# HenryHZY/VL-PET

Hardware: AMD Instinct MI355X
Metric: multitask samples/sec (BART-base, r=96) (higher is better)
Workload: dtype bf16

## Files before the change

vl-pet_amd/csrc/attn.hip:

```cpp
#include <cstdlib>
#include "common.h"
#include "kernels.h"

#define AT_LD 72
#define AT_ROW (AT_LD * 2)
#define AT_NW 4
#define LOG2E 1.4426950408889634f

typedef short v4s16_t __attribute__((ext_vector_type(4)));
typedef short v8s16_t __attribute__((ext_vector_type(8)));

__device__ __forceinline__ float fast_exp2(float x) { return __builtin_amdgcn_exp2f(x); }

__device__ __forceinline__ uint32_t hash32(uint32_t x) {
    x ^= x >> 16; x *= 0x7feb352dU; x ^= x >> 15; x *= 0x846ca68bU; x ^= x >> 16;
    return x;
}
__device__ __forceinline__ uint32_t row_key(uint64_t seed, int64_t row) {
    const uint32_t k = hash32((uint32_t)seed ^ hash32((uint32_t)(seed >> 32) + (uint32_t)((uint64_t)row >> 32)));
    return hash32(k + (uint32_t)row);
}
__device__ __forceinline__ uint32_t hash_elem(uint32_t x) {
    x ^= x >> 16; x *= 0x7feb352dU; x ^= x >> 15;
    return __builtin_amdgcn_alignbit(x, x, 16) * 0x846ca68bU;
}
__device__ __forceinline__ bool keep_elem(uint32_t rk, int j, uint32_t thr) { return hash_elem(rk + (uint32_t)j * 0x9E3779B9U) >= thr; }

__device__ __forceinline__ bf16x8 tr_acc_order(const uint8_t* img, int kb, int cb, int lane) {
    const int g = lane >> 4, sl = lane & 15;
    const uint8_t* p = img + (size_t)(kb + 4 * (g >> 1) + (sl >> 2)) * AT_ROW + (cb + 16 * (g & 1) + 4 * (sl & 3)) * 2;
    typedef __attribute__((address_space(3))) v4s16_t lds_v4;
    const v4s16_t lo = __builtin_amdgcn_ds_read_tr16_b64_v4i16((lds_v4*)(p));
    const v4s16_t hi = __builtin_amdgcn_ds_read_tr16_b64_v4i16((lds_v4*)(p + 8 * AT_ROW));
    const v8s16_t r = {lo[0], lo[1], lo[2], lo[3], hi[0], hi[1], hi[2], hi[3]};
    return __builtin_bit_cast(bf16x8, r);
}
__device__ __forceinline__ bf16x8 nat_frag(const uint8_t* img, int row, int ks, int hh) {
    return *reinterpret_cast<const bf16x8*>(img + (size_t)row * AT_ROW + (16 * ks + 8 * hh) * 2);
}
__device__ __forceinline__ bf16x8 acc_frag(const f32x16& t, int u) {
    bf16x8 f;
#pragma unroll
    for (int j = 0; j < 8; ++j) f[j] = (__bf16)t[8 * u + j];
    return f;
}
__device__ __forceinline__ void stage_image(uint8_t* img, const __bf16* src, int64_t rs, int n_rows, int rows_pad, int tid, int nthreads) {
    const u32x4 z = {0u, 0u, 0u, 0u};
    for (int idx = tid; idx < rows_pad * 8; idx += nthreads) {
        const int row = idx >> 3, pc = idx & 7;
        u32x4 v = z;
        if (row < n_rows) v = __builtin_nontemporal_load(reinterpret_cast<const u32x4*>(src + (int64_t)row * rs + pc * 8));
        *reinterpret_cast<u32x4*>(img + (size_t)row * AT_ROW + pc * 16) = v;
    }
}
template <int NIMG, int MAXP>
__device__ __forceinline__ void stage_images(uint8_t* const* img, const __bf16* const* src, const int* n_rows, const int* rows_pad,
                                             const int64_t* rs, int tid, int nthreads) {
    u32x4 v[NIMG][MAXP];
#pragma unroll
    for (int g = 0; g < NIMG; ++g)
#pragma unroll
        for (int c = 0; c < MAXP; ++c) {
            const int idx = tid + c * nthreads, row = idx >> 3, pc = idx & 7;
            const int rr = row < n_rows[g] ? row : n_rows[g] - 1;
            v[g][c] = __builtin_nontemporal_load(reinterpret_cast<const u32x4*>(src[g] + (int64_t)rr * rs[g] + pc * 8));
        }
    const u32x4 z = {0u, 0u, 0u, 0u};
#pragma unroll
    for (int g = 0; g < NIMG; ++g)
#pragma unroll
        for (int c = 0; c < MAXP; ++c) {
            const int idx = tid + c * nthreads, row = idx >> 3, pc = idx & 7;
            if (row < rows_pad[g]) *reinterpret_cast<u32x4*>(img[g] + (size_t)row * AT_ROW + pc * 16) = row < n_rows[g] ? v[g][c] : z;
        }
}
#define AT_SROW 144
#define AT_STG (16 * AT_SROW)
__device__ __forceinline__ void store_rows_T(uint8_t* stg, const f32x16& t0, const f32x16& t1, __bf16* dst, int64_t rs,
                                             int row0, int n_rows, int lane) {
    const int m = lane & 31, hh = lane >> 5;
    typedef __bf16 bf16x4_t __attribute__((ext_vector_type(4)));
#pragma unroll
    for (int half = 0; half < 2; ++half) {
        if ((m >> 4) == half) {
#pragma unroll
            for (int dt = 0; dt < 2; ++dt) {
                const f32x16& t = dt ? t1 : t0;
#pragma unroll
                for (int q = 0; q < 4; ++q) {
                    bf16x4_t w;
#pragma unroll
                    for (int e = 0; e < 4; ++e) w[e] = (__bf16)t[4 * q + e];
                    *reinterpret_cast<bf16x4_t*>(stg + (size_t)(m & 15) * AT_SROW + (32 * dt + 8 * q + 4 * hh) * 2) = w;
                }
            }
        }
        asm volatile("" ::: "memory");
        u32x4 v[2];
#pragma unroll
        for (int c = 0; c < 2; ++c) {
            const int idx = lane + 64 * c, row = idx >> 3, pc = idx & 7;
            v[c] = *reinterpret_cast<const u32x4*>(stg + (size_t)row * AT_SROW + pc * 16);
        }
        asm volatile("" ::: "memory");
#pragma unroll
        for (int c = 0; c < 2; ++c) {
            const int idx = lane + 64 * c, row = 16 * half + (idx >> 3), pc = idx & 7;
            if (row0 + row < n_rows) *reinterpret_cast<u32x4*>(dst + (int64_t)(row0 + row) * rs + pc * 8) = v[c];
        }
    }
}

__device__ __forceinline__ f32x16 bias_tile(const float* brow, float inv_scale) {
    f32x16 t;
#pragma unroll
    for (int q4 = 0; q4 < 4; ++q4) {
        const f32x4 bv = *reinterpret_cast<const f32x4*>(brow + 8 * q4);
#pragma unroll
        for (int e = 0; e < 4; ++e) t[4 * q4 + e] = bv[e] * inv_scale;
    }
    return t;
}

#define AT_FW 2

struct AttnLds {
    __host__ __device__ static constexpr size_t fwd_wave_bytes(int Lkp) { return (size_t)Lkp * AT_ROW + (size_t)AT_STG + (size_t)Lkp * 4; }
    static size_t fwd_bytes(int Lkp) { return (size_t)AT_FW * fwd_wave_bytes(Lkp); }
    static size_t bwd_bytes(int Lqp, int Lkp) {
        return bwd_bytes_nw(Lqp, Lkp, AT_NW);
    }
    static size_t bwd_bytes_nw(int Lqp, int Lkp, int nw) {
        return (size_t)2 * (Lqp + Lkp) * AT_ROW + (size_t)nw * AT_STG + (size_t)Lqp * 12 + (size_t)Lkp * 4;
    }
};

__device__ __forceinline__ float key_bias(const AttnArgs& a, const uint8_t* km, int key) {
    return (key < a.Lk && (km == nullptr || km[key] != 0)) ? 0.f : -INFINITY;
}

template <int T, bool BIAS>
__global__ __launch_bounds__(AT_FW * 64, (T <= 2 ? 3 : 2)) void attn_fwd_kernel(AttnArgs a) {
    extern __shared__ __attribute__((aligned(16))) uint8_t smem[];
    const int tid = threadIdx.x, lane = tid & 63, wave = __builtin_amdgcn_readfirstlane(tid >> 6);
    const int bh = blockIdx.x * AT_FW + wave;
    if (bh >= a.B * a.H) return;
    const uint64_t seed = a.thr ? vlpet_eff_seed(a.seed, a.seed_ctr) : 0;
    const int b = bh / a.H, h = bh % a.H;
    const int m = lane & 31, hh = lane >> 5;
    constexpr int Lkp = 32 * T;
    const int64_t rs = (int64_t)a.H * 64, rq = a.ld_q, rk = a.ld_kv, rv = a.ld_v;
    const __bf16* qb_ = a.q + (int64_t)b * a.Lq * rq + h * 64;
    const __bf16* kb_ = a.k + (int64_t)b * a.Lk * rk + h * 64;
    const __bf16* vb_ = a.v + (int64_t)b * a.Lk * rv + h * 64;
    __bf16* ob_ = a.o + (int64_t)b * a.Lq * rs + h * 64;
    const uint8_t* km = a.key_mask ? a.key_mask + (int64_t)b * a.Lk : nullptr;
    uint8_t* Vs = smem + (size_t)wave * AttnLds::fwd_wave_bytes(Lkp);
    uint8_t* stg = Vs + (size_t)Lkp * AT_ROW;
    float* kval = reinterpret_cast<float*>(stg + AT_STG);
#pragma unroll
    for (int c = 0; c < (Lkp + 63) / 64; ++c)
        if (lane + 64 * c < Lkp) kval[lane + 64 * c] = key_bias(a, km, lane + 64 * c);
    const int coff = a.causal ? a.Lk - a.Lq : (1 << 20);

    bf16x8 kf[T][4];
#pragma unroll
    for (int t = 0; t < T; ++t) {
        const int j = 32 * t + m, jk = j < a.Lk ? j : a.Lk - 1;
#pragma unroll
        for (int ks = 0; ks < 4; ++ks) kf[t][ks] = *reinterpret_cast<const bf16x8*>(kb_ + (int64_t)jk * rk + 16 * ks + 8 * hh);
    }
    stage_image(Vs, vb_, rv, a.Lk, Lkp, lane, 64);

    const float sc2 = a.scale * LOG2E;
    const int NQB = (a.Lq + 31) >> 5;
    for (int qb = 0; qb < NQB; ++qb) {
        const int i = 32 * qb + m;
        const int iq = i < a.Lq ? i : a.Lq - 1;
        bf16x8 qf[4];
#pragma unroll
        for (int ks = 0; ks < 4; ++ks) qf[ks] = *reinterpret_cast<const bf16x8*>(qb_ + (int64_t)iq * rq + 16 * ks + 8 * hh);
        f32x16 st[T];
#pragma unroll
        for (int t = 0; t < T; ++t) {
            if constexpr (BIAS) st[t] = bias_tile(a.bias + ((int64_t)h * (32 * NQB) + i) * Lkp + 32 * t + 4 * hh, 1.0f / a.scale);
            else st[t] = zero16();
#pragma unroll
            for (int ks = 0; ks < 4; ++ks) st[t] = mfma32(kf[t][ks], qf[ks], st[t]);
        }
        float mx = -INFINITY;
        const int ic = i + coff - 4 * hh;
#pragma unroll
        for (int t = 0; t < T; ++t) {
#pragma unroll
            for (int q4 = 0; q4 < 4; ++q4) {
                const f32x4 kv = *reinterpret_cast<const f32x4*>(kval + 32 * t + 8 * q4 + 4 * hh);
#pragma unroll
                for (int e = 0; e < 4; ++e) {
                    const int r = 4 * q4 + e;
                    float s = fmaf(st[t][r], sc2, kv[e]);
                    s = 32 * t + e + 8 * q4 > ic ? -INFINITY : s;
                    st[t][r] = s;
                    mx = fmaxf(mx, s);
                }
            }
        }
        mx = fmaxf(mx, __shfl_xor(mx, 32));
        if (mx == -INFINITY) mx = 0.f;
        float sum = 0.f;
#pragma unroll
        for (int t = 0; t < T; ++t) {
#pragma unroll
            for (int r = 0; r < 16; ++r) { const float p = fast_exp2(st[t][r] - mx); st[t][r] = p; sum += p; }
        }
        sum += __shfl_xor(sum, 32);
        const float inv = sum > 0.f ? 1.0f / sum : 0.f;
        if (hh == 0 && i < a.Lq) a.lse[((int64_t)b * a.H + h) * a.Lq + i] = sum > 0.f ? mx + log2f(sum) : INFINITY;
        const uint32_t rk = row_key(seed, ((int64_t)b * a.H + h) * a.Lq + iq);
        const float inv_keep = a.thr ? a.inv_keep : 1.0f;
        f32x16 ot0 = zero16(), ot1 = zero16();
#pragma unroll
        for (int t = 0; t < T; ++t) {
            if (a.keep_out != nullptr && a.thr != 0) {
#pragma unroll
                for (int r = 0; r < 16; ++r) {
                    const int key = 32 * t + (r & 3) + 8 * (r >> 2) + 4 * hh;
                    if (i < a.Lq && key < a.Lk)
                        a.keep_out[(((int64_t)b * a.H + h) * a.Lq + i) * a.Lk + key] = keep_elem(rk, key, a.thr) ? 1 : 0;
                }
            }
            const uint32_t kg0 = rk + (uint32_t)(32 * t + 4 * hh) * 0x9E3779B9U;
#pragma unroll
            for (int r = 0; r < 16; ++r) {
                const int ir = (r & 3) + 8 * (r >> 2);
                const bool kp = hash_elem(kg0 + (uint32_t)ir * 0x9E3779B9U) >= a.thr;
                st[t][r] = kp ? st[t][r] * inv * inv_keep : 0.f;
            }
#pragma unroll
            for (int u = 0; u < 2; ++u) {
                const bf16x8 pf = acc_frag(st[t], u);
                ot0 = mfma32(tr_acc_order(Vs, 32 * t + 16 * u, 0, lane), pf, ot0);
                ot1 = mfma32(tr_acc_order(Vs, 32 * t + 16 * u, 32, lane), pf, ot1);
            }
        }
        store_rows_T(stg, ot0, ot1, ob_, rs, 32 * qb, a.Lq, lane);
    }
}

enum { IMG_Q = 0, IMG_D = 1, IMG_K = 2, IMG_V = 3 };
struct BwdCtx {
    const float* rowt;
    const float* kval;
    int Lqp;
    float sc2, scale, inv_keep;
    uint32_t thr;
    int coff;
};
__device__ __forceinline__ BwdCtx bwd_ctx(const AttnArgs& a, const float* rowt, const float* kval, int Lqp) {
    BwdCtx c;
    c.rowt = rowt; c.kval = kval; c.Lqp = Lqp;
    c.sc2 = a.scale * LOG2E; c.scale = a.scale; c.inv_keep = a.thr ? a.inv_keep : 1.0f; c.thr = a.thr;
    c.coff = a.causal ? a.Lk - a.Lq : (1 << 20);
    return c;
}

template <class R, bool BIAS>
__device__ __forceinline__ void bwd_k_unit(const AttnArgs& a, const BwdCtx& c, const R& rd0, int t, int NQB, int Lqp, int Lkp, int h, int lane,
                                           f32x16& dv0, f32x16& dv1, f32x16& dk0, f32x16& dk1) {
    const int m = lane & 31, hh = lane >> 5;
    const int key = 32 * t + m;
    const float kb = c.kval[key];
    const uint32_t kg = (uint32_t)key * 0x9E3779B9U;
    const int kc = key - c.coff - 4 * hh;
    for (int qb = 0; qb < NQB; ++qb) {
        const R rd = rd0.fresh();
        f32x16 s, dp = zero16();
        if constexpr (BIAS) s = bias_tile(a.bias_t + ((int64_t)h * Lkp + key) * Lqp + 32 * qb + 4 * hh, 1.0f / a.scale);
        else s = zero16();
#pragma unroll
        for (int ks = 0; ks < 4; ++ks) {
            s = mfma32(rd.nat(IMG_Q, qb, ks), rd.nat(IMG_K, t, ks), s);
            dp = mfma32(rd.nat(IMG_D, qb, ks), rd.nat(IMG_V, t, ks), dp);
        }
        const int kcq = kc - 32 * qb;
        const float* rtp = c.rowt + 32 * qb + 4 * hh;
#pragma unroll
        for (int q4 = 0; q4 < 4; ++q4) {
            __builtin_amdgcn_sched_barrier(0);
            const f32x4 ls = *reinterpret_cast<const f32x4*>(rtp + 8 * q4);
            const f32x4 dl = *reinterpret_cast<const f32x4*>(rtp + c.Lqp + 8 * q4);
            const f32x4 rk = *reinterpret_cast<const f32x4*>(rtp + 2 * c.Lqp + 8 * q4);
#pragma unroll
            for (int e = 0; e < 4; ++e) {
                const int r = 4 * q4 + e, ir = e + 8 * q4;
                float x = fmaf(s[r], c.sc2, kb - ls[e]);
                x = kcq > ir ? -INFINITY : x;
                const float p = fast_exp2(x);
                const bool kp = hash_elem(__float_as_uint(rk[e]) + kg) >= c.thr;
                const float g = kp ? dp[r] * c.inv_keep : 0.f;
                s[r] = kp ? p * c.inv_keep : 0.f;
                dp[r] = p * (g - dl[e]) * c.scale;
            }
        }
#pragma unroll
        for (int u = 0; u < 2; ++u) {
            const bf16x8 pf = acc_frag(s, u), sf = acc_frag(dp, u);
            dv0 = mfma32(rd.tr(IMG_D, 2 * qb + u, 0), pf, dv0);
            dv1 = mfma32(rd.tr(IMG_D, 2 * qb + u, 1), pf, dv1);
            dk0 = mfma32(rd.tr(IMG_Q, 2 * qb + u, 0), sf, dk0);
            dk1 = mfma32(rd.tr(IMG_Q, 2 * qb + u, 1), sf, dk1);
        }
    }
}
template <class R, bool BIAS>
__device__ __forceinline__ void bwd_q_unit(const AttnArgs& a, const BwdCtx& c, const R& rd0, int qb, int T, int Lqp, int Lkp, int h, int lane,
                                           f32x16& dq0, f32x16& dq1) {
    const int m = lane & 31, hh = lane >> 5;
    const int i = 32 * qb + m;
    bf16x8 qf[4], df[4];
#pragma unroll
    for (int ks = 0; ks < 4; ++ks) { qf[ks] = rd0.nat(IMG_Q, qb, ks); df[ks] = rd0.nat(IMG_D, qb, ks); }
    const float l2 = c.rowt[i], dl = c.rowt[c.Lqp + i];
    const uint32_t rkey = __float_as_uint(c.rowt[2 * c.Lqp + i]);
    const int ic = i + c.coff - 4 * hh;
    for (int t = 0; t < T; ++t) {
        const R rd = rd0.fresh();
        f32x16 s, dp = zero16();
        if constexpr (BIAS) s = bias_tile(a.bias + ((int64_t)h * Lqp + i) * Lkp + 32 * t + 4 * hh, 1.0f / a.scale);
        else s = zero16();
#pragma unroll
        for (int ks = 0; ks < 4; ++ks) {
            s = mfma32(rd.nat(IMG_K, t, ks), qf[ks], s);
            dp = mfma32(rd.nat(IMG_V, t, ks), df[ks], dp);
        }
        const float* kvp = c.kval + 32 * t + 4 * hh;
        const uint32_t kg0 = rkey + (uint32_t)(32 * t + 4 * hh) * 0x9E3779B9U;
        const int ict = ic - 32 * t;
#pragma unroll
        for (int q4 = 0; q4 < 4; ++q4) {
            __builtin_amdgcn_sched_barrier(0);
            const f32x4 kv = *reinterpret_cast<const f32x4*>(kvp + 8 * q4);
#pragma unroll
            for (int e = 0; e < 4; ++e) {
                const int r = 4 * q4 + e, ir = e + 8 * q4;
                float x = fmaf(s[r], c.sc2, kv[e] - l2);
                x = ir > ict ? -INFINITY : x;
                const float p = fast_exp2(x);
                const bool kp = hash_elem(kg0 + (uint32_t)ir * 0x9E3779B9U) >= c.thr;
                const float g = kp ? dp[r] * c.inv_keep : 0.f;
                dp[r] = p * (g - dl) * c.scale;
            }
        }
#pragma unroll
        for (int u = 0; u < 2; ++u) {
            const bf16x8 sf = acc_frag(dp, u);
            dq0 = mfma32(rd.tr(IMG_K, 2 * t + u, 0), sf, dq0);
            dq1 = mfma32(rd.tr(IMG_K, 2 * t + u, 1), sf, dq1);
        }
    }
}
struct PadRd {
    const uint8_t* img[4];
    int m, hh, lane;
    __device__ __forceinline__ PadRd fresh() const { PadRd r = *this; asm volatile("" : "+v"(r.m), "+v"(r.lane)); return r; }
    __device__ __forceinline__ bf16x8 nat(int im, int tile, int ks) const { return nat_frag(img[im], 32 * tile + m, ks, hh); }
    __device__ __forceinline__ bf16x8 tr(int im, int g16, int dt) const { return tr_acc_order(img[im], 16 * g16, 32 * dt, lane); }
};
template <int OCC, int NW = AT_NW, bool BIAS = false>
__global__ __launch_bounds__(NW * 64, OCC) void attn_bwd_kernel(AttnArgs a) {
    extern __shared__ __attribute__((aligned(16))) uint8_t smem[];
    const int bh = blockIdx.x, b = bh / a.H, h = bh % a.H;
    const int tid = threadIdx.x, lane = tid & 63, wave = __builtin_amdgcn_readfirstlane(tid >> 6);
    const uint64_t seed = a.thr ? vlpet_eff_seed(a.seed, a.seed_ctr) : 0;
    const int m = lane & 31, hh = lane >> 5;
    const int Lkp = (a.Lk + 31) & ~31, T = Lkp >> 5;
    const int Lqp = (a.Lq + 31) & ~31, NQB = Lqp >> 5;
    const int64_t rs = (int64_t)a.H * 64, rq = a.ld_q, rk = a.ld_kv, rv = a.ld_v;
    const int64_t ooff = (int64_t)b * a.Lq * rs + h * 64;
    const int64_t qoff = (int64_t)b * a.Lq * rq + h * 64, koff = (int64_t)b * a.Lk * rk + h * 64;
    const int64_t voff = (int64_t)b * a.Lk * rv + h * 64;
    const uint8_t* km = a.key_mask ? a.key_mask + (int64_t)b * a.Lk : nullptr;
    uint8_t* Qs = smem;
    uint8_t* Ds = Qs + (size_t)Lqp * AT_ROW;
    uint8_t* Ks = Ds + (size_t)Lqp * AT_ROW;
    uint8_t* Vs = Ks + (size_t)Lkp * AT_ROW;
    uint8_t* stg = Vs + (size_t)Lkp * AT_ROW + (size_t)wave * AT_STG;
    float* rowt = reinterpret_cast<float*>(Vs + (size_t)Lkp * AT_ROW + (size_t)NW * AT_STG);
    float* kval = rowt + 3 * Lqp;

    {
        bf16x8 xo[2][2], xd[2][2];
#pragma unroll
        for (int c = 0; c < 2; ++c) {
            const int idx = tid + c * NW * 64, row = idx >> 2, part = idx & 3;
            const int rr = row < a.Lq ? row : a.Lq - 1;
#pragma unroll
            for (int e = 0; e < 2; ++e) {
                xo[c][e] = __builtin_nontemporal_load(reinterpret_cast<const bf16x8*>(a.o + ooff + (int64_t)rr * rs + 16 * part + 8 * e));
                xd[c][e] = __builtin_nontemporal_load(reinterpret_cast<const bf16x8*>(a.dout + ooff + (int64_t)rr * rs + 16 * part + 8 * e));
            }
        }
        if (tid < Lkp) kval[tid] = key_bias(a, km, tid);
        uint8_t* const imgs[4] = {Qs, Ds, Ks, Vs};
        const __bf16* const srcs[4] = {a.q + qoff, a.dout + ooff, a.k + koff, a.v + voff};
        const int nr[4] = {a.Lq, a.Lq, a.Lk, a.Lk}, rp[4] = {Lqp, Lqp, Lkp, Lkp};
        const int64_t rss[4] = {rq, rs, rk, rv};
        stage_images<4, (NW == 6 ? 3 : 4)>(imgs, srcs, nr, rp, rss, tid, NW * 64);
#pragma unroll
        for (int c = 0; c < 2; ++c) {
            const int idx = tid + c * NW * 64, row = idx >> 2, part = idx & 3;
            float acc = 0.f;
#pragma unroll
            for (int e = 0; e < 2; ++e)
#pragma unroll
                for (int j = 0; j < 8; ++j) acc += (float)xo[c][e][j] * (float)xd[c][e][j];
            acc += __shfl_xor(acc, 1);
            acc += __shfl_xor(acc, 2);
            if (part == 0 && row < Lqp) {
                const bool live = row < a.Lq;
                rowt[row] = live ? a.lse[((int64_t)b * a.H + h) * a.Lq + row] : INFINITY;
                rowt[Lqp + row] = live ? acc : 0.f;
                rowt[2 * Lqp + row] = __uint_as_float(row_key(seed, ((int64_t)b * a.H + h) * a.Lq + (live ? row : a.Lq - 1)));
            }
        }
    }
    __syncthreads();

    const BwdCtx c = bwd_ctx(a, rowt, kval, Lqp);
    PadRd rd;
    rd.img[IMG_Q] = Qs; rd.img[IMG_D] = Ds; rd.img[IMG_K] = Ks; rd.img[IMG_V] = Vs;
    rd.m = m; rd.hh = hh; rd.lane = lane;
    for (int un = (a.dbg & 1) ? T + NQB : wave; un < T + NQB; un += NW) {
        if (un < T) {
            f32x16 dv0 = zero16(), dv1 = zero16(), dk0 = zero16(), dk1 = zero16();
            if (!(a.dbg & 8)) bwd_k_unit<PadRd, BIAS>(a, c, rd, un, NQB, Lqp, Lkp, h, lane, dv0, dv1, dk0, dk1);
            if (a.dbg & 4) { if (dv0[0] + dv1[1] + dk0[2] + dk1[3] == 1.2345f) a.dv[0] = (__bf16)1.f; continue; }
            store_rows_T(stg, dv0, dv1, a.dv + voff, rv, 32 * un, a.Lk, lane);
            store_rows_T(stg, dk0, dk1, a.dk + koff, rk, 32 * un, a.Lk, lane);
        } else {
            f32x16 dq0 = zero16(), dq1 = zero16();
            if (!(a.dbg & 8)) bwd_q_unit<PadRd, BIAS>(a, c, rd, un - T, T, Lqp, Lkp, h, lane, dq0, dq1);
            if (a.dbg & 4) { if (dq0[0] + dq1[1] == 1.2345f) a.dq[0] = (__bf16)1.f; continue; }
            store_rows_T(stg, dq0, dq1, a.dq + qoff, rq, 32 * (un - T), a.Lq, lane);
        }
    }
}

size_t attn_lds_bytes(int Lq, int Lk, int bwd) {
    const int Lqp = (Lq + 31) & ~31, Lkp = (Lk + 31) & ~31;
    return bwd ? AttnLds::bwd_bytes(Lqp, Lkp) : AttnLds::fwd_bytes(Lkp);
}

template <int T, bool BIAS>
static hipError_t launch_attn_fwd_tb(const AttnArgs& a, hipStream_t stream) {
    const size_t lds = AttnLds::fwd_bytes(32 * T);
    auto kern = attn_fwd_kernel<T, BIAS>;
    hipError_t e = hipFuncSetAttribute(reinterpret_cast<const void*>(kern), hipFuncAttributeMaxDynamicSharedMemorySize, (int)lds);
    if (e != hipSuccess) return e;
    const unsigned pairs = (unsigned)(a.B * a.H);
    hipLaunchKernelGGL(kern, dim3((pairs + AT_FW - 1) / AT_FW), dim3(AT_FW * 64), lds, stream, a);
    return hipGetLastError();
}

template <int T>
static hipError_t launch_attn_fwd_t(const AttnArgs& a, hipStream_t stream) {
    return a.bias != nullptr ? launch_attn_fwd_tb<T, true>(a, stream) : launch_attn_fwd_tb<T, false>(a, stream);
}

hipError_t launch_attn(const AttnArgs& a_in, bool bwd, hipStream_t stream) {
    AttnArgs a = a_in;
    a.dbg = VLPET_IS_DEBUG_BUILD ? vlpet_tuning().dbg : 0;
    if (!bwd) {
        switch ((a.Lk + 31) >> 5) {
            case 1: return launch_attn_fwd_t<1>(a, stream);
            case 2: return launch_attn_fwd_t<2>(a, stream);
            case 3: return launch_attn_fwd_t<3>(a, stream);
            case 4: return launch_attn_fwd_t<4>(a, stream);
            default: return hipErrorInvalidValue;
        }
    }
    const int Lqp = (a.Lq + 31) & ~31, Lkp = (a.Lk + 31) & ~31;
    const int units = (Lqp >> 5) + (Lkp >> 5);
    const int occ_env = vlpet_tuning().attn_occ;
    const int nw_env = vlpet_tuning().attn_nw;
    const size_t lds6 = AttnLds::bwd_bytes_nw(Lqp, Lkp, 6);
    if (nw_env == 6 && (units == 5 || units == 6) && 2 * (lds6 + 512) <= (size_t)160 * 1024) {
        auto k6 = attn_bwd_kernel<3, 6>;
        hipError_t e6 = hipFuncSetAttribute(reinterpret_cast<const void*>(k6), hipFuncAttributeMaxDynamicSharedMemorySize, (int)lds6);
        if (e6 != hipSuccess) return e6;
        hipLaunchKernelGGL(k6, dim3((unsigned)(a.B * a.H)), dim3(6 * 64), lds6, stream, a);
        return hipGetLastError();
    }
    const size_t lds = attn_lds_bytes(a.Lq, a.Lk, 1);
    if (a.bias != nullptr) {
        const bool o3 = occ_env == 3 || (occ_env != 2 && 3 * (lds + 512) <= (size_t)160 * 1024);
        const void* kb = o3 ? reinterpret_cast<const void*>(attn_bwd_kernel<3, AT_NW, true>) : reinterpret_cast<const void*>(attn_bwd_kernel<2, AT_NW, true>);
        hipError_t eb = hipFuncSetAttribute(kb, hipFuncAttributeMaxDynamicSharedMemorySize, (int)lds);
        if (eb != hipSuccess) return eb;
        if (o3) hipLaunchKernelGGL((attn_bwd_kernel<3, AT_NW, true>), dim3((unsigned)(a.B * a.H)), dim3(AT_NW * 64), lds, stream, a);
        else hipLaunchKernelGGL((attn_bwd_kernel<2, AT_NW, true>), dim3((unsigned)(a.B * a.H)), dim3(AT_NW * 64), lds, stream, a);
        return hipGetLastError();
    }
    const bool occ3 = occ_env == 3 || (occ_env != 2 && 3 * (lds + 512) <= (size_t)160 * 1024);
    const void* kern = occ3 ? reinterpret_cast<const void*>(attn_bwd_kernel<3>) : reinterpret_cast<const void*>(attn_bwd_kernel<2>);
    hipError_t e = hipFuncSetAttribute(kern, hipFuncAttributeMaxDynamicSharedMemorySize, (int)lds);
    if (e != hipSuccess) return e;
    if (occ3) hipLaunchKernelGGL(attn_bwd_kernel<3>, dim3((unsigned)(a.B * a.H)), dim3(AT_NW * 64), lds, stream, a);
    else hipLaunchKernelGGL(attn_bwd_kernel<2>, dim3((unsigned)(a.B * a.H)), dim3(AT_NW * 64), lds, stream, a);
    return hipGetLastError();
}
```

vl-pet_amd/csrc/tuning.h:

```cpp
#pragma once
#include <cstdlib>

struct VlpetTuning {
    int rg = 0;
    int bwd2 = 1;
    int bwd3 = -1;
    int bwd3_units = 0;
    int bwd3_form = 1;
    int k4_waves4 = 0;
    int wgrad_wgs = 0;
    int wgrad_tr = 1;
    int wgrad_stream = 1;
    int wgrad_nstg = 3;
    int wgs_mode = 0;
    int attn_occ = 0;
    int attn_nw = 0;
    int dz2 = 1;
    int dz2_fsplit = 0;
    int dz6 = 1;
    int k4_wgrad2 = 1;
    int ng2 = 1;
    int fwd2p = -1;
    int cols_red = 1;
    int dbg = 0;
};

#ifdef VLPET_DEBUG
inline const VlpetTuning& vlpet_tuning() {
    static const VlpetTuning t = [] {
        VlpetTuning v;
        auto rd = [](const char* n, int& dst) { if (const char* e = getenv(n)) dst = atoi(e); };
        rd("VLPET_RG", v.rg); rd("VLPET_BWD2", v.bwd2); rd("VLPET_BWD3", v.bwd3); rd("VLPET_BWD3_UNITS", v.bwd3_units);
        rd("VLPET_BWD3_FORM", v.bwd3_form); rd("VLPET_K4_WAVES4", v.k4_waves4); rd("VLPET_WGRAD_WGS", v.wgrad_wgs);
        rd("VLPET_WGRAD_TR", v.wgrad_tr); rd("VLPET_WGRAD_STREAM", v.wgrad_stream); rd("VLPET_WGRAD_NSTG", v.wgrad_nstg);
        rd("VLPET_WGS_MODE", v.wgs_mode); rd("VLPET_ATTN_OCC", v.attn_occ); rd("VLPET_ATTN_NW", v.attn_nw); rd("VLPET_DBG", v.dbg); rd("VLPET_DZ2", v.dz2); rd("VLPET_DZ6", v.dz6); rd("VLPET_DZ2_FSPLIT", v.dz2_fsplit); rd("VLPET_K4_WGRAD2", v.k4_wgrad2); rd("VLPET_NG2", v.ng2); rd("VLPET_FWD2P", v.fwd2p); rd("VLPET_COLS_RED", v.cols_red);
        return v;
    }();
    return t;
}
#define VLPET_IS_DEBUG_BUILD 1
#else
inline const VlpetTuning& vlpet_tuning() { static const VlpetTuning t{}; return t; }
#define VLPET_IS_DEBUG_BUILD 0
#endif
```

Measured before the change: 30280.

## Compute attention backward dS once in LDS and reuse for dQ

The attention backward kernel used to recompute the score and dropout tile in separate key-block and query-block units. It now has each wave evaluate its (query block, key tile) pairs once, store the bf16 dS tiles in LDS, and build dQ from transposed LDS reads of those tiles. When there are fewer key tiles than waves, idle waves take over the last query block and hand P/dS off through shared memory. A separate units kernel handles the 32x32 case, and the NW=6 variant and its tuning knob are removed. The exchange is a larger LDS footprint per block, which can lower occupancy, plus an extra barrier between the compute and contraction phases.

```diff
diff --git a/vl-pet_amd/csrc/attn.hip b/vl-pet_amd/csrc/attn.hip
--- a/vl-pet_amd/csrc/attn.hip
+++ b/vl-pet_amd/csrc/attn.hip
@@ -76,6 +76,7 @@
 }
 #define AT_SROW 144
 #define AT_STG (16 * AT_SROW)
+#define AT_TILE 2048
 __device__ __forceinline__ void store_rows_T(uint8_t* stg, const f32x16& t0, const f32x16& t1, __bf16* dst, int64_t rs,
                                              int row0, int n_rows, int lane) {
     const int m = lane & 31, hh = lane >> 5;
@@ -127,11 +128,15 @@
 struct AttnLds {
     __host__ __device__ static constexpr size_t fwd_wave_bytes(int Lkp) { return (size_t)Lkp * AT_ROW + (size_t)AT_STG + (size_t)Lkp * 4; }
     static size_t fwd_bytes(int Lkp) { return (size_t)AT_FW * fwd_wave_bytes(Lkp); }
+    __host__ __device__ static constexpr size_t bwd_v_bytes(int Lkp) {
+        return (size_t)Lkp * AT_ROW > (size_t)AT_NW * AT_STG ? (size_t)Lkp * AT_ROW : (size_t)AT_NW * AT_STG;
+    }
+    __host__ __device__ static constexpr int bwd_p_tiles(int Lqp, int Lkp) { return (Lkp < 32 * AT_NW && Lqp >= 64) ? Lkp / 32 : 0; }
+    static constexpr bool bwd_single_pair(int Lqp, int Lkp) { return Lqp == 32 && Lkp == 32; }
     static size_t bwd_bytes(int Lqp, int Lkp) {
-        return bwd_bytes_nw(Lqp, Lkp, AT_NW);
-    }
-    static size_t bwd_bytes_nw(int Lqp, int Lkp, int nw) {
-        return (size_t)2 * (Lqp + Lkp) * AT_ROW + (size_t)nw * AT_STG + (size_t)Lqp * 12 + (size_t)Lkp * 4;
+        if (bwd_single_pair(Lqp, Lkp)) return (size_t)4 * 32 * AT_ROW + (size_t)2 * AT_STG + (size_t)32 * 16;
+        return (size_t)(2 * Lqp + Lkp) * AT_ROW + bwd_v_bytes(Lkp) + (size_t)((Lqp / 32) * (Lkp / 32) + bwd_p_tiles(Lqp, Lkp)) * AT_TILE
+               + (size_t)Lqp * 12 + (size_t)Lkp * 4;
     }
 };
 
@@ -263,57 +268,220 @@
     c.coff = a.causal ? a.Lk - a.Lq : (1 << 20);
     return c;
 }
-
-template <class R, bool BIAS>
-__device__ __forceinline__ void bwd_k_unit(const AttnArgs& a, const BwdCtx& c, const R& rd0, int t, int NQB, int Lqp, int Lkp, int h, int lane,
-                                           f32x16& dv0, f32x16& dv1, f32x16& dk0, f32x16& dk1) {
+struct PadRd {
+    const uint8_t* img[4];
+    int m, hh, lane;
+    __device__ __forceinline__ PadRd fresh() const { PadRd r = *this; asm volatile("" : "+v"(r.m), "+v"(r.lane)); return r; }
+    __device__ __forceinline__ bf16x8 nat(int im, int tile, int ks) const { return nat_frag(img[im], 32 * tile + m, ks, hh); }
+    __device__ __forceinline__ bf16x8 tr(int im, int g16, int dt) const { return tr_acc_order(img[im], 16 * g16, 32 * dt, lane); }
+};
+
+template <bool BIAS>
+__device__ __forceinline__ void bwd_eval_pair(const AttnArgs& a, const BwdCtx& c, const PadRd& rd0, int qb, int t, int Lqp, int Lkp, int h,
+                                              int lane, bf16x8 (&pf)[2], bf16x8 (&sf)[2]) {
     const int m = lane & 31, hh = lane >> 5;
     const int key = 32 * t + m;
     const float kb = c.kval[key];
     const uint32_t kg = (uint32_t)key * 0x9E3779B9U;
-    const int kc = key - c.coff - 4 * hh;
-    for (int qb = 0; qb < NQB; ++qb) {
-        const R rd = rd0.fresh();
-        f32x16 s, dp = zero16();
-        if constexpr (BIAS) s = bias_tile(a.bias_t + ((int64_t)h * Lkp + key) * Lqp + 32 * qb + 4 * hh, 1.0f / a.scale);
-        else s = zero16();
-#pragma unroll
-        for (int ks = 0; ks < 4; ++ks) {
-            s = mfma32(rd.nat(IMG_Q, qb, ks), rd.nat(IMG_K, t, ks), s);
-            dp = mfma32(rd.nat(IMG_D, qb, ks), rd.nat(IMG_V, t, ks), dp);
-        }
-        const int kcq = kc - 32 * qb;
-        const float* rtp = c.rowt + 32 * qb + 4 * hh;
-#pragma unroll
-        for (int q4 = 0; q4 < 4; ++q4) {
-            __builtin_amdgcn_sched_barrier(0);
-            const f32x4 ls = *reinterpret_cast<const f32x4*>(rtp + 8 * q4);
-            const f32x4 dl = *reinterpret_cast<const f32x4*>(rtp + c.Lqp + 8 * q4);
-            const f32x4 rk = *reinterpret_cast<const f32x4*>(rtp + 2 * c.Lqp + 8 * q4);
-#pragma unroll
-            for (int e = 0; e < 4; ++e) {
-                const int r = 4 * q4 + e, ir = e + 8 * q4;
-                float x = fmaf(s[r], c.sc2, kb - ls[e]);
-                x = kcq > ir ? -INFINITY : x;
-                const float p = fast_exp2(x);
-                const bool kp = hash_elem(__float_as_uint(rk[e]) + kg) >= c.thr;
-                const float g = kp ? dp[r] * c.inv_keep : 0.f;
-                s[r] = kp ? p * c.inv_keep : 0.f;
-                dp[r] = p * (g - dl[e]) * c.scale;
-            }
-        }
-#pragma unroll
-        for (int u = 0; u < 2; ++u) {
-            const bf16x8 pf = acc_frag(s, u), sf = acc_frag(dp, u);
-            dv0 = mfma32(rd.tr(IMG_D, 2 * qb + u, 0), pf, dv0);
-            dv1 = mfma32(rd.tr(IMG_D, 2 * qb + u, 1), pf, dv1);
-            dk0 = mfma32(rd.tr(IMG_Q, 2 * qb + u, 0), sf, dk0);
-            dk1 = mfma32(rd.tr(IMG_Q, 2 * qb + u, 1), sf, dk1);
-        }
-    }
-}
-template <class R, bool BIAS>
-__device__ __forceinline__ void bwd_q_unit(const AttnArgs& a, const BwdCtx& c, const R& rd0, int qb, int T, int Lqp, int Lkp, int h, int lane,
+    const int kcq = key - c.coff - 4 * hh - 32 * qb;
+    const PadRd rd = rd0.fresh();
+    f32x16 s, dp = zero16();
+    if constexpr (BIAS) s = bias_tile(a.bias_t + ((int64_t)h * Lkp + key) * Lqp + 32 * qb + 4 * hh, 1.0f / a.scale);
+    else s = zero16();
+#pragma unroll
+    for (int ks = 0; ks < 4; ++ks) {
+        s = mfma32(rd.nat(IMG_Q, qb, ks), rd.nat(IMG_K, t, ks), s);
+        dp = mfma32(rd.nat(IMG_D, qb, ks), rd.nat(IMG_V, t, ks), dp);
+    }
+    const float* rtp = c.rowt + 32 * qb + 4 * hh;
+#pragma unroll
+    for (int q4 = 0; q4 < 4; ++q4) {
+        __builtin_amdgcn_sched_barrier(0);
+        const f32x4 ls = *reinterpret_cast<const f32x4*>(rtp + 8 * q4);
+        const f32x4 dl = *reinterpret_cast<const f32x4*>(rtp + c.Lqp + 8 * q4);
+        const f32x4 rk = *reinterpret_cast<const f32x4*>(rtp + 2 * c.Lqp + 8 * q4);
+#pragma unroll
+        for (int e = 0; e < 4; ++e) {
+            const int r = 4 * q4 + e, ir = e + 8 * q4;
+            float x = fmaf(s[r], c.sc2, kb - ls[e]);
+            x = kcq > ir ? -INFINITY : x;
+            const float p = fast_exp2(x);
+            const bool kp = hash_elem(__float_as_uint(rk[e]) + kg) >= c.thr;
+            const float g = kp ? dp[r] * c.inv_keep : 0.f;
+            s[r] = kp ? p * c.inv_keep : 0.f;
+            dp[r] = p * (g - dl[e]) * c.scale;
+        }
+    }
+#pragma unroll
+    for (int u = 0; u < 2; ++u) { pf[u] = acc_frag(s, u); sf[u] = acc_frag(dp, u); }
+}
+__device__ __forceinline__ void bwd_contract_kv(const PadRd& rd, int qb, const bf16x8 (&pf)[2], const bf16x8 (&sf)[2],
+                                                f32x16& dv0, f32x16& dv1, f32x16& dk0, f32x16& dk1) {
+#pragma unroll
+    for (int u = 0; u < 2; ++u) {
+        dv0 = mfma32(rd.tr(IMG_D, 2 * qb + u, 0), pf[u], dv0);
+        dv1 = mfma32(rd.tr(IMG_D, 2 * qb + u, 1), pf[u], dv1);
+        dk0 = mfma32(rd.tr(IMG_Q, 2 * qb + u, 0), sf[u], dk0);
+        dk1 = mfma32(rd.tr(IMG_Q, 2 * qb + u, 1), sf[u], dk1);
+    }
+}
+__device__ __forceinline__ void bwd_stage(const AttnArgs& a, int b, int h, int tid, int Lqp, int Lkp, uint8_t* Qs, uint8_t* Ds, uint8_t* Ks,
+                                          uint8_t* Vs, float* rowt, float* kval) {
+    constexpr int NW = AT_NW;
+    const uint64_t seed = a.thr ? vlpet_eff_seed(a.seed, a.seed_ctr) : 0;
+    const int64_t rs = (int64_t)a.H * 64, rq = a.ld_q, rk = a.ld_kv, rv = a.ld_v;
+    const int64_t ooff = (int64_t)b * a.Lq * rs + h * 64;
+    const int64_t qoff = (int64_t)b * a.Lq * rq + h * 64, koff = (int64_t)b * a.Lk * rk + h * 64, voff = (int64_t)b * a.Lk * rv + h * 64;
+    const uint8_t* km = a.key_mask ? a.key_mask + (int64_t)b * a.Lk : nullptr;
+    bf16x8 xo[2][2], xd[2][2];
+#pragma unroll
+    for (int c = 0; c < 2; ++c) {
+        const int idx = tid + c * NW * 64, row = idx >> 2, part = idx & 3;
+        const int rr = row < a.Lq ? row : a.Lq - 1;
+#pragma unroll
+        for (int e = 0; e < 2; ++e) {
+            xo[c][e] = __builtin_nontemporal_load(reinterpret_cast<const bf16x8*>(a.o + ooff + (int64_t)rr * rs + 16 * part + 8 * e));
+            xd[c][e] = __builtin_nontemporal_load(reinterpret_cast<const bf16x8*>(a.dout + ooff + (int64_t)rr * rs + 16 * part + 8 * e));
+        }
+    }
+    if (tid < Lkp) kval[tid] = key_bias(a, km, tid);
+    uint8_t* const imgs[4] = {Qs, Ds, Ks, Vs};
+    const __bf16* const srcs[4] = {a.q + qoff, a.dout + ooff, a.k + koff, a.v + voff};
+    const int nr[4] = {a.Lq, a.Lq, a.Lk, a.Lk}, rp[4] = {Lqp, Lqp, Lkp, Lkp};
+    const int64_t rss[4] = {rq, rs, rk, rv};
+    stage_images<4, 4>(imgs, srcs, nr, rp, rss, tid, NW * 64);
+#pragma unroll
+    for (int c = 0; c < 2; ++c) {
+        const int idx = tid + c * NW * 64, row = idx >> 2, part = idx & 3;
+        float acc = 0.f;
+#pragma unroll
+        for (int e = 0; e < 2; ++e)
+#pragma unroll
+            for (int j = 0; j < 8; ++j) acc += (float)xo[c][e][j] * (float)xd[c][e][j];
+        acc += __shfl_xor(acc, 1);
+        acc += __shfl_xor(acc, 2);
+        if (part == 0 && row < Lqp) {
+            const bool live = row < a.Lq;
+            rowt[row] = live ? a.lse[((int64_t)b * a.H + h) * a.Lq + row] : INFINITY;
+            rowt[Lqp + row] = live ? acc : 0.f;
+            rowt[2 * Lqp + row] = __uint_as_float(row_key(seed, ((int64_t)b * a.H + h) * a.Lq + (live ? row : a.Lq - 1)));
+        }
+    }
+}
+typedef __bf16 bf16x4_t __attribute__((ext_vector_type(4)));
+__device__ __forceinline__ void ds_tile_put(uint8_t* tile, const bf16x8 (&sf)[2], int m, int hh) {
+#pragma unroll
+    for (int u = 0; u < 2; ++u) {
+        const bf16x4_t lo = {sf[u][0], sf[u][1], sf[u][2], sf[u][3]}, hi = {sf[u][4], sf[u][5], sf[u][6], sf[u][7]};
+        *reinterpret_cast<bf16x4_t*>(tile + m * 64 + (16 * u + 4 * hh) * 2) = lo;
+        *reinterpret_cast<bf16x4_t*>(tile + m * 64 + (16 * u + 8 + 4 * hh) * 2) = hi;
+    }
+}
+__device__ __forceinline__ void ds_tile_get(const uint8_t* tile, bf16x8 (&sf)[2], int m, int hh) {
+#pragma unroll
+    for (int u = 0; u < 2; ++u) {
+        const bf16x4_t lo = *reinterpret_cast<const bf16x4_t*>(tile + m * 64 + (16 * u + 4 * hh) * 2);
+        const bf16x4_t hi = *reinterpret_cast<const bf16x4_t*>(tile + m * 64 + (16 * u + 8 + 4 * hh) * 2);
+        sf[u] = bf16x8{lo[0], lo[1], lo[2], lo[3], hi[0], hi[1], hi[2], hi[3]};
+    }
+}
+__device__ __forceinline__ bf16x8 ds_tile_tr(const uint8_t* tile, int u, int lane) {
+    const int g = lane >> 4, sl = lane & 15;
+    const uint8_t* p = tile + (16 * u + 4 * (g >> 1) + (sl >> 2)) * 64 + (16 * (g & 1) + 4 * (sl & 3)) * 2;
+    typedef __attribute__((address_space(3))) v4s16_t lds_v4;
+    const v4s16_t lo = __builtin_amdgcn_ds_read_tr16_b64_v4i16((lds_v4*)(p));
+    const v4s16_t hi = __builtin_amdgcn_ds_read_tr16_b64_v4i16((lds_v4*)(p + 8 * 64));
+    const v8s16_t r = {lo[0], lo[1], lo[2], lo[3], hi[0], hi[1], hi[2], hi[3]};
+    return __builtin_bit_cast(bf16x8, r);
+}
+
+template <int OCC, bool BIAS = false>
+__global__ __launch_bounds__(AT_NW * 64, OCC) void attn_bwd_kernel(AttnArgs a) {
+    extern __shared__ __attribute__((aligned(16))) uint8_t smem[];
+    constexpr int NW = AT_NW;
+    const int bh = blockIdx.x, b = bh / a.H, h = bh % a.H;
+    const int tid = threadIdx.x, lane = tid & 63, wave = __builtin_amdgcn_readfirstlane(tid >> 6);
+    const int m = lane & 31, hh = lane >> 5;
+    const int Lkp = (a.Lk + 31) & ~31, T = Lkp >> 5;
+    const int Lqp = (a.Lq + 31) & ~31, NQB = Lqp >> 5;
+    const int64_t rq = a.ld_q, rk = a.ld_kv, rv = a.ld_v;
+    const int64_t qoff = (int64_t)b * a.Lq * rq + h * 64, koff = (int64_t)b * a.Lk * rk + h * 64;
+    const int64_t voff = (int64_t)b * a.Lk * rv + h * 64;
+    uint8_t* Qs = smem;
+    uint8_t* Ds = Qs + (size_t)Lqp * AT_ROW;
+    uint8_t* Ks = Ds + (size_t)Lqp * AT_ROW;
+    uint8_t* Vs = Ks + (size_t)Lkp * AT_ROW;
+    uint8_t* dSt = Vs + AttnLds::bwd_v_bytes(Lkp);
+    uint8_t* Pt = dSt + (size_t)T * NQB * AT_TILE;
+    float* rowt = reinterpret_cast<float*>(Pt + (size_t)AttnLds::bwd_p_tiles(Lqp, Lkp) * AT_TILE);
+    float* kval = rowt + 3 * Lqp;
+
+    bwd_stage(a, b, h, tid, Lqp, Lkp, Qs, Ds, Ks, Vs, rowt, kval);
+    __syncthreads();
+
+    const BwdCtx c = bwd_ctx(a, rowt, kval, Lqp);
+    PadRd rd;
+    rd.img[IMG_Q] = Qs; rd.img[IMG_D] = Ds; rd.img[IMG_K] = Ks; rd.img[IMG_V] = Vs;
+    rd.m = m; rd.hh = hh; rd.lane = lane;
+    const bool comp = !(a.dbg & 9);
+    const bool help = T < NW && NQB >= 2;
+    const int nown = help ? NQB - 1 : NQB;
+    f32x16 dv0 = zero16(), dv1 = zero16(), dk0 = zero16(), dk1 = zero16();
+    bf16x8 pf[2], sf[2];
+    if (comp) {
+        if (wave < T) {
+            for (int qb = 0; qb < nown; ++qb) {
+                bwd_eval_pair<BIAS>(a, c, rd, qb, wave, Lqp, Lkp, h, lane, pf, sf);
+                ds_tile_put(dSt + (size_t)(wave * NQB + qb) * AT_TILE, sf, m, hh);
+                if (qb + 1 < nown) bwd_contract_kv(rd.fresh(), qb, pf, sf, dv0, dv1, dk0, dk1);
+            }
+        } else if (help) {
+            for (int t = wave - T; t < T; t += NW - T) {
+                bwd_eval_pair<BIAS>(a, c, rd, NQB - 1, t, Lqp, Lkp, h, lane, pf, sf);
+                ds_tile_put(dSt + (size_t)(t * NQB + NQB - 1) * AT_TILE, sf, m, hh);
+#pragma unroll
+                for (int u = 0; u < 2; ++u) *reinterpret_cast<bf16x8*>(Pt + (size_t)t * AT_TILE + (u * 64 + lane) * 16) = pf[u];
+            }
+        }
+    }
+    __syncthreads();
+    if (a.dbg & 1) return;
+    uint8_t* stg = Vs + (size_t)wave * AT_STG;
+    if (wave < T) {
+        if (comp) bwd_contract_kv(rd.fresh(), nown - 1, pf, sf, dv0, dv1, dk0, dk1);
+        if (comp && help) {
+#pragma unroll
+            for (int u = 0; u < 2; ++u) pf[u] = *reinterpret_cast<const bf16x8*>(Pt + (size_t)wave * AT_TILE + (u * 64 + lane) * 16);
+            ds_tile_get(dSt + (size_t)(wave * NQB + NQB - 1) * AT_TILE, sf, m, hh);
+            bwd_contract_kv(rd.fresh(), NQB - 1, pf, sf, dv0, dv1, dk0, dk1);
+        }
+        if (a.dbg & 4) { if (dv0[0] + dv1[1] + dk0[2] + dk1[3] == 1.2345f) a.dv[0] = (__bf16)1.f; }
+        else {
+            store_rows_T(stg, dv0, dv1, a.dv + voff, rv, 32 * wave, a.Lk, lane);
+            store_rows_T(stg, dk0, dk1, a.dk + koff, rk, 32 * wave, a.Lk, lane);
+        }
+    }
+    const int qo = NW - 1 - wave;
+    if (qo < NQB) {
+        f32x16 dq0 = zero16(), dq1 = zero16();
+        if (comp) {
+            for (int t = 0; t < T; ++t) {
+                const PadRd r2 = rd.fresh();
+#pragma unroll
+                for (int u = 0; u < 2; ++u) {
+                    const bf16x8 sb = ds_tile_tr(dSt + (size_t)(t * NQB + qo) * AT_TILE, u, r2.lane);
+                    dq0 = mfma32(r2.tr(IMG_K, 2 * t + u, 0), sb, dq0);
+                    dq1 = mfma32(r2.tr(IMG_K, 2 * t + u, 1), sb, dq1);
+                }
+            }
+        }
+        if (a.dbg & 4) { if (dq0[0] + dq1[1] == 1.2345f) a.dq[0] = (__bf16)1.f; }
+        else store_rows_T(stg, dq0, dq1, a.dq + qoff, rq, 32 * qo, a.Lq, lane);
+    }
+}
+
+template <bool BIAS>
+__device__ __forceinline__ void bwd_q_unit(const AttnArgs& a, const BwdCtx& c, const PadRd& rd0, int qb, int T, int Lqp, int Lkp, int h, int lane,
                                            f32x16& dq0, f32x16& dq1) {
     const int m = lane & 31, hh = lane >> 5;
     const int i = 32 * qb + m;
@@ -324,7 +492,7 @@
     const uint32_t rkey = __float_as_uint(c.rowt[2 * c.Lqp + i]);
     const int ic = i + c.coff - 4 * hh;
     for (int t = 0; t < T; ++t) {
-        const R rd = rd0.fresh();
+        const PadRd rd = rd0.fresh();
         f32x16 s, dp = zero16();
         if constexpr (BIAS) s = bias_tile(a.bias + ((int64_t)h * Lqp + i) * Lkp + 32 * t + 4 * hh, 1.0f / a.scale);
         else s = zero16();
@@ -359,90 +527,41 @@
         }
     }
 }
-struct PadRd {
-    const uint8_t* img[4];
-    int m, hh, lane;
-    __device__ __forceinline__ PadRd fresh() const { PadRd r = *this; asm volatile("" : "+v"(r.m), "+v"(r.lane)); return r; }
-    __device__ __forceinline__ bf16x8 nat(int im, int tile, int ks) const { return nat_frag(img[im], 32 * tile + m, ks, hh); }
-    __device__ __forceinline__ bf16x8 tr(int im, int g16, int dt) const { return tr_acc_order(img[im], 16 * g16, 32 * dt, lane); }
-};
-template <int OCC, int NW = AT_NW, bool BIAS = false>
-__global__ __launch_bounds__(NW * 64, OCC) void attn_bwd_kernel(AttnArgs a) {
+template <bool BIAS>
+__global__ __launch_bounds__(AT_NW * 64, 3) void attn_bwd_units_kernel(AttnArgs a) {
     extern __shared__ __attribute__((aligned(16))) uint8_t smem[];
     const int bh = blockIdx.x, b = bh / a.H, h = bh % a.H;
     const int tid = threadIdx.x, lane = tid & 63, wave = __builtin_amdgcn_readfirstlane(tid >> 6);
-    const uint64_t seed = a.thr ? vlpet_eff_seed(a.seed, a.seed_ctr) : 0;
-    const int m = lane & 31, hh = lane >> 5;
-    const int Lkp = (a.Lk + 31) & ~31, T = Lkp >> 5;
-    const int Lqp = (a.Lq + 31) & ~31, NQB = Lqp >> 5;
-    const int64_t rs = (int64_t)a.H * 64, rq = a.ld_q, rk = a.ld_kv, rv = a.ld_v;
-    const int64_t ooff = (int64_t)b * a.Lq * rs + h * 64;
-    const int64_t qoff = (int64_t)b * a.Lq * rq + h * 64, koff = (int64_t)b * a.Lk * rk + h * 64;
-    const int64_t voff = (int64_t)b * a.Lk * rv + h * 64;
-    const uint8_t* km = a.key_mask ? a.key_mask + (int64_t)b * a.Lk : nullptr;
+    constexpr int Lqp = 32, Lkp = 32;
     uint8_t* Qs = smem;
     uint8_t* Ds = Qs + (size_t)Lqp * AT_ROW;
     uint8_t* Ks = Ds + (size_t)Lqp * AT_ROW;
     uint8_t* Vs = Ks + (size_t)Lkp * AT_ROW;
     uint8_t* stg = Vs + (size_t)Lkp * AT_ROW + (size_t)wave * AT_STG;
-    float* rowt = reinterpret_cast<float*>(Vs + (size_t)Lkp * AT_ROW + (size_t)NW * AT_STG);
+    float* rowt = reinterpret_cast<float*>(Vs + (size_t)Lkp * AT_ROW + (size_t)2 * AT_STG);
     float* kval = rowt + 3 * Lqp;
-
-    {
-        bf16x8 xo[2][2], xd[2][2];
-#pragma unroll
-        for (int c = 0; c < 2; ++c) {
-            const int idx = tid + c * NW * 64, row = idx >> 2, part = idx & 3;
-            const int rr = row < a.Lq ? row : a.Lq - 1;
-#pragma unroll
-            for (int e = 0; e < 2; ++e) {
-                xo[c][e] = __builtin_nontemporal_load(reinterpret_cast<const bf16x8*>(a.o + ooff + (int64_t)rr * rs + 16 * part + 8 * e));
-                xd[c][e] = __builtin_nontemporal_load(reinterpret_cast<const bf16x8*>(a.dout + ooff + (int64_t)rr * rs + 16 * part + 8 * e));
-            }
-        }
-        if (tid < Lkp) kval[tid] = key_bias(a, km, tid);
-        uint8_t* const imgs[4] = {Qs, Ds, Ks, Vs};
-        const __bf16* const srcs[4] = {a.q + qoff, a.dout + ooff, a.k + koff, a.v + voff};
-        const int nr[4] = {a.Lq, a.Lq, a.Lk, a.Lk}, rp[4] = {Lqp, Lqp, Lkp, Lkp};
-        const int64_t rss[4] = {rq, rs, rk, rv};
-        stage_images<4, (NW == 6 ? 3 : 4)>(imgs, srcs, nr, rp, rss, tid, NW * 64);
-#pragma unroll
-        for (int c = 0; c < 2; ++c) {
-            const int idx = tid + c * NW * 64, row = idx >> 2, part = idx & 3;
-            float acc = 0.f;
-#pragma unroll
-            for (int e = 0; e < 2; ++e)
-#pragma unroll
-                for (int j = 0; j < 8; ++j) acc += (float)xo[c][e][j] * (float)xd[c][e][j];
-            acc += __shfl_xor(acc, 1);
-            acc += __shfl_xor(acc, 2);
-            if (part == 0 && row < Lqp) {
-                const bool live = row < a.Lq;
-                rowt[row] = live ? a.lse[((int64_t)b * a.H + h) * a.Lq + row] : INFINITY;
-                rowt[Lqp + row] = live ? acc : 0.f;
-                rowt[2 * Lqp + row] = __uint_as_float(row_key(seed, ((int64_t)b * a.H + h) * a.Lq + (live ? row : a.Lq - 1)));
-            }
-        }
-    }
+    bwd_stage(a, b, h, tid, Lqp, Lkp, Qs, Ds, Ks, Vs, rowt, kval);
     __syncthreads();
-
+    if (wave >= 2 || (a.dbg & 1)) return;
     const BwdCtx c = bwd_ctx(a, rowt, kval, Lqp);
     PadRd rd;
     rd.img[IMG_Q] = Qs; rd.img[IMG_D] = Ds; rd.img[IMG_K] = Ks; rd.img[IMG_V] = Vs;
-    rd.m = m; rd.hh = hh; rd.lane = lane;
-    for (int un = (a.dbg & 1) ? T + NQB : wave; un < T + NQB; un += NW) {
-        if (un < T) {
-            f32x16 dv0 = zero16(), dv1 = zero16(), dk0 = zero16(), dk1 = zero16();
-            if (!(a.dbg & 8)) bwd_k_unit<PadRd, BIAS>(a, c, rd, un, NQB, Lqp, Lkp, h, lane, dv0, dv1, dk0, dk1);
-            if (a.dbg & 4) { if (dv0[0] + dv1[1] + dk0[2] + dk1[3] == 1.2345f) a.dv[0] = (__bf16)1.f; continue; }
-            store_rows_T(stg, dv0, dv1, a.dv + voff, rv, 32 * un, a.Lk, lane);
-            store_rows_T(stg, dk0, dk1, a.dk + koff, rk, 32 * un, a.Lk, lane);
-        } else {
-            f32x16 dq0 = zero16(), dq1 = zero16();
-            if (!(a.dbg & 8)) bwd_q_unit<PadRd, BIAS>(a, c, rd, un - T, T, Lqp, Lkp, h, lane, dq0, dq1);
-            if (a.dbg & 4) { if (dq0[0] + dq1[1] == 1.2345f) a.dq[0] = (__bf16)1.f; continue; }
-            store_rows_T(stg, dq0, dq1, a.dq + qoff, rq, 32 * (un - T), a.Lq, lane);
-        }
+    rd.m = lane & 31; rd.hh = lane >> 5; rd.lane = lane;
+    if (wave == 0) {
+        f32x16 dv0 = zero16(), dv1 = zero16(), dk0 = zero16(), dk1 = zero16();
+        if (!(a.dbg & 8)) {
+            bf16x8 pf[2], sf[2];
+            bwd_eval_pair<BIAS>(a, c, rd, 0, 0, Lqp, Lkp, h, lane, pf, sf);
+            bwd_contract_kv(rd.fresh(), 0, pf, sf, dv0, dv1, dk0, dk1);
+        }
+        if (a.dbg & 4) { if (dv0[0] + dv1[1] + dk0[2] + dk1[3] == 1.2345f) a.dv[0] = (__bf16)1.f; return; }
+        store_rows_T(stg, dv0, dv1, a.dv + (int64_t)b * a.Lk * a.ld_v + h * 64, a.ld_v, 0, a.Lk, lane);
+        store_rows_T(stg, dk0, dk1, a.dk + (int64_t)b * a.Lk * a.ld_kv + h * 64, a.ld_kv, 0, a.Lk, lane);
+    } else {
+        f32x16 dq0 = zero16(), dq1 = zero16();
+        if (!(a.dbg & 8)) bwd_q_unit<BIAS>(a, c, rd, 0, 1, Lqp, Lkp, h, lane, dq0, dq1);
+        if (a.dbg & 4) { if (dq0[0] + dq1[1] == 1.2345f) a.dq[0] = (__bf16)1.f; return; }
+        store_rows_T(stg, dq0, dq1, a.dq + (int64_t)b * a.Lq * a.ld_q + h * 64, a.ld_q, 0, a.Lq, lane);
     }
 }
 
@@ -479,33 +598,19 @@
             default: return hipErrorInvalidValue;
         }
     }
-    const int Lqp = (a.Lq + 31) & ~31, Lkp = (a.Lk + 31) & ~31;
-    const int units = (Lqp >> 5) + (Lkp >> 5);
     const int occ_env = vlpet_tuning().attn_occ;
-    const int nw_env = vlpet_tuning().attn_nw;
-    const size_t lds6 = AttnLds::bwd_bytes_nw(Lqp, Lkp, 6);
-    if (nw_env == 6 && (units == 5 || units == 6) && 2 * (lds6 + 512) <= (size_t)160 * 1024) {
-        auto k6 = attn_bwd_kernel<3, 6>;
-        hipError_t e6 = hipFuncSetAttribute(reinterpret_cast<const void*>(k6), hipFuncAttributeMaxDynamicSharedMemorySize, (int)lds6);
-        if (e6 != hipSuccess) return e6;
-        hipLaunchKernelGGL(k6, dim3((unsigned)(a.B * a.H)), dim3(6 * 64), lds6, stream, a);
+    const size_t lds = attn_lds_bytes(a.Lq, a.Lk, 1);
+    const bool occ3 = occ_env == 3 || (occ_env != 2 && 3 * (lds + 512) <= (size_t)160 * 1024);
+    const bool biased = a.bias != nullptr;
+    if (AttnLds::bwd_single_pair((a.Lq + 31) & ~31, (a.Lk + 31) & ~31)) {
+        auto ku = biased ? attn_bwd_units_kernel<true> : attn_bwd_units_kernel<false>;
+        hipLaunchKernelGGL(ku, dim3((unsigned)(a.B * a.H)), dim3(AT_NW * 64), lds, stream, a);
         return hipGetLastError();
     }
-    const size_t lds = attn_lds_bytes(a.Lq, a.Lk, 1);
-    if (a.bias != nullptr) {
-        const bool o3 = occ_env == 3 || (occ_env != 2 && 3 * (lds + 512) <= (size_t)160 * 1024);
-        const void* kb = o3 ? reinterpret_cast<const void*>(attn_bwd_kernel<3, AT_NW, true>) : reinterpret_cast<const void*>(attn_bwd_kernel<2, AT_NW, true>);
-        hipError_t eb = hipFuncSetAttribute(kb, hipFuncAttributeMaxDynamicSharedMemorySize, (int)lds);
-        if (eb != hipSuccess) return eb;
-        if (o3) hipLaunchKernelGGL((attn_bwd_kernel<3, AT_NW, true>), dim3((unsigned)(a.B * a.H)), dim3(AT_NW * 64), lds, stream, a);
-        else hipLaunchKernelGGL((attn_bwd_kernel<2, AT_NW, true>), dim3((unsigned)(a.B * a.H)), dim3(AT_NW * 64), lds, stream, a);
-        return hipGetLastError();
-    }
-    const bool occ3 = occ_env == 3 || (occ_env != 2 && 3 * (lds + 512) <= (size_t)160 * 1024);
-    const void* kern = occ3 ? reinterpret_cast<const void*>(attn_bwd_kernel<3>) : reinterpret_cast<const void*>(attn_bwd_kernel<2>);
-    hipError_t e = hipFuncSetAttribute(kern, hipFuncAttributeMaxDynamicSharedMemorySize, (int)lds);
+    auto kern = occ3 ? (biased ? attn_bwd_kernel<3, true> : attn_bwd_kernel<3, false>)
+                     : (biased ? attn_bwd_kernel<2, true> : attn_bwd_kernel<2, false>);
+    hipError_t e = hipFuncSetAttribute(reinterpret_cast<const void*>(kern), hipFuncAttributeMaxDynamicSharedMemorySize, (int)lds);
     if (e != hipSuccess) return e;
-    if (occ3) hipLaunchKernelGGL(attn_bwd_kernel<3>, dim3((unsigned)(a.B * a.H)), dim3(AT_NW * 64), lds, stream, a);
-    else hipLaunchKernelGGL(attn_bwd_kernel<2>, dim3((unsigned)(a.B * a.H)), dim3(AT_NW * 64), lds, stream, a);
+    hipLaunchKernelGGL(kern, dim3((unsigned)(a.B * a.H)), dim3(AT_NW * 64), lds, stream, a);
     return hipGetLastError();
 }
diff --git a/vl-pet_amd/csrc/tuning.h b/vl-pet_amd/csrc/tuning.h
--- a/vl-pet_amd/csrc/tuning.h
+++ b/vl-pet_amd/csrc/tuning.h
@@ -14,7 +14,6 @@
     int wgrad_nstg = 3;
     int wgs_mode = 0;
     int attn_occ = 0;
-    int attn_nw = 0;
     int dz2 = 1;
     int dz2_fsplit = 0;
     int dz6 = 1;
@@ -33,7 +32,7 @@
         rd("VLPET_RG", v.rg); rd("VLPET_BWD2", v.bwd2); rd("VLPET_BWD3", v.bwd3); rd("VLPET_BWD3_UNITS", v.bwd3_units);
         rd("VLPET_BWD3_FORM", v.bwd3_form); rd("VLPET_K4_WAVES4", v.k4_waves4); rd("VLPET_WGRAD_WGS", v.wgrad_wgs);
         rd("VLPET_WGRAD_TR", v.wgrad_tr); rd("VLPET_WGRAD_STREAM", v.wgrad_stream); rd("VLPET_WGRAD_NSTG", v.wgrad_nstg);
-        rd("VLPET_WGS_MODE", v.wgs_mode); rd("VLPET_ATTN_OCC", v.attn_occ); rd("VLPET_ATTN_NW", v.attn_nw); rd("VLPET_DBG", v.dbg); rd("VLPET_DZ2", v.dz2); rd("VLPET_DZ6", v.dz6); rd("VLPET_DZ2_FSPLIT", v.dz2_fsplit); rd("VLPET_K4_WGRAD2", v.k4_wgrad2); rd("VLPET_NG2", v.ng2); rd("VLPET_FWD2P", v.fwd2p); rd("VLPET_COLS_RED", v.cols_red);
+        rd("VLPET_WGS_MODE", v.wgs_mode); rd("VLPET_ATTN_OCC", v.attn_occ); rd("VLPET_DBG", v.dbg); rd("VLPET_DZ2", v.dz2); rd("VLPET_DZ6", v.dz6); rd("VLPET_DZ2_FSPLIT", v.dz2_fsplit); rd("VLPET_K4_WGRAD2", v.k4_wgrad2); rd("VLPET_NG2", v.ng2); rd("VLPET_FWD2P", v.fwd2p); rd("VLPET_COLS_RED", v.cols_red);
         return v;
     }();
     return t;
```

Measured after the change: 30540 (median of 6 runs). About the same (+0.9%).
